# VITA-Group/mm-hand

Measured on AMD Instinct MI355X. Metric: 256x256 hand images/sec (G+D step), higher is better.
Workload: dtype f32; 1 GPU; RHD-shaped 256x256, per-GPU batch 32, fp32 (Winograd F(6x6,3x3) on the 3x3 stack), G(9 PATBlocks, ngf64)+D_PB+D_PP+L1/perceptual/GAN+Adam, --norm instance, dropout on; VGG19[:4] weights: random-init (seed 1234): NOT the reference's pretrained objective; global_batch=32, parallelism=dp1

## Files before the change

### include/mmhand_hip.h

```cpp
#ifndef MMHAND_HIP_H
#define MMHAND_HIP_H

#include <stddef.h>
#include <stdint.h>

#ifdef __cplusplus
extern "C" {
#endif
#pragma GCC visibility push(default)

typedef void* mmh_stream_t;

enum { MMH_PAD_ZERO = 0, MMH_PAD_REFLECT = 1 };
enum { MMH_ACT_NONE = 0, MMH_ACT_RELU = 1, MMH_ACT_TANH = 2 };
enum { MMH_F32 = 0, MMH_BF16 = 1, MMH_FP16 = 2 };

typedef struct mmh_conv_desc {
    int32_t B, H, W;
    int32_t Cin, Cout;
    int32_t kh, kw;
    int32_t stride;
    int32_t pad;
    int32_t pad_mode;
    int32_t Ho, Wo;
// ... 1 lines not shown
    int32_t dtype;
} mmh_conv_desc;

const char* mmh_last_error(void);
int mmh_version(void);
int mmh_set_option(const char* key, int value);


int mmh_conv2d_fprop(const mmh_conv_desc* d, const void* x, const void* w,
                     const void* bias, void* y, int act, mmh_stream_t s);

int mmh_conv2d_fprop_stats_chunks(const mmh_conv_desc* d);
int mmh_conv2d_fprop_stats(const mmh_conv_desc* d, const void* x, const void* w, const void* bias,
                           void* y, void* stats, mmh_stream_t s);
int mmh_dgrad_s2_halo_supported(const mmh_conv_desc* d, int dx_cs);

int mmh_conv2d_dgrad(const mmh_conv_desc* d, const void* dy, const void* w,
                     void* dx, int dx_cs, mmh_stream_t s);

size_t mmh_conv2d_dgrad_folded_ws_bytes(const mmh_conv_desc* d);
int mmh_conv2d_dgrad_folded(const mmh_conv_desc* d, const void* dy, const void* w,
                            void* dx, void* ws, size_t ws_bytes, mmh_stream_t s);

int mmh_wino_weights(const void* w, int Cin, int Cout, int flip_transpose, int tile, int dtype,
                     void* U, mmh_stream_t s);
int mmh_wino_input(const void* x, int B, int H, int W, int C, int reflect, int tile, int dtype,
                   void* V, mmh_stream_t s);
int mmh_wino_dy(const void* dy, int B, int H, int W, int C, int tile, int dtype, void* Yh,
                mmh_stream_t s);
int mmh_wino_input_dy(const void* dy, int B, int H, int W, int C, int tile, int dtype, void* V,
// ... 390 lines not shown
```

### mmhand_amd/csrc/common.h

```cpp
#pragma once
#include <hip/hip_runtime.h>
#include <cstdarg>
#include <cstdio>
#include <cstdint>
#include "../../include/mmhand_hip.h"

namespace mmh {

char* err_buf();
int fail(const char* fmt, ...);

inline int check_launch(const char* what) {
    hipError_t e = hipGetLastError();
    if (e != hipSuccess) return fail("%s: %s", what, hipGetErrorString(e));
    return 0;
}

inline hipStream_t as_stream(mmh_stream_t s) { return reinterpret_cast<hipStream_t>(s); }

inline int64_t cdiv(int64_t a, int64_t b) { return (a + b - 1) / b; }

int wino6_weights(const float* w, float* U, int Cin, int Cout, int flip_transpose, hipStream_t st);
int wino6_weights_multi(const long long* table, int n, long long total_blocks, hipStream_t st);
int wino6_input(const float* x, float* V, int B, int H, int W, int C, int reflect, int xcd, hipStream_t st);
// ... 5 lines not shown
                        const uint32_t* drows, hipStream_t st);
int wino6_input_dy_normbwd(const float* g, const float* x, float* V, float* Yh, int B, int H, int W, int C, int xcd,
                           int fold, const float* mean, const float* invstd, const float* gamma, const float* s1,
                           const float* s2, double count, const float* scale, const float* shift,
                           const uint32_t* drows, int groups, int relu, float drop_p, hipStream_t st);
int wino6_input_dy(const float* dy, float* V, float* Yh, int B, int H, int W, int C, int xcd, int fold,
                   hipStream_t st);
int wino6_dw(const float* dU, float* dw, int Cin, int Cout, int accumulate, hipStream_t st);
bool wgrad_lp16t_supported(const mmh_conv_desc* d);
int wgrad_lp16t_splits(const mmh_conv_desc* d);
int launch_wgrad_lp16t(const mmh_conv_desc* d, const void* x16, const void* dy16, float* slab, const void* zeros,
                       hipStream_t st);
bool dgrad_s2_halo_ok(const mmh_conv_desc* d, int dx_cs, int act);
int launch_dgrad_s2_halo(const mmh_conv_desc* d, const void* dy, const void* w, const void* bias, void* dx, int dx_cs,
                         int act, hipStream_t st);
extern int g_dgrad_s2_halo, g_dgrad_s2_dbg;
bool wgrad_s2_strip_ok(const mmh_conv_desc* d);
size_t wgrad_s2_strip_ws_bytes(const mmh_conv_desc* d);
int launch_wgrad_s2_strip(const mmh_conv_desc* d, const void* x, const void* dy, void* dw, void* ws, size_t ws_bytes,
                          int accumulate, hipStream_t st);
extern int g_wgrad_s2_strip;
bool stem_f32_ok(const mmh_conv_desc* d);
int stem_f32_stats_chunks(const mmh_conv_desc* d);
int launch_stem_f32(const mmh_conv_desc* d, const void* x, const void* w, const void* bias, void* y, int act, float* stats,
                    hipStream_t st);
extern int g_stem_f32, g_stem_f32_dbg, g_stem_f32_levels;
bool wino_wgrad_dma_ok(int64_t tiles, int Cin, int Cout, int nbatch);
size_t wino_wgrad_dma_ws_bytes(int64_t tiles, int Cin, int Cout, int nbatch);
int launch_wino_wgrad_dma(const float* V, const float* Yh, int64_t tiles, int Cin, int Cout, int nbatch, float* ws, float* dU,
                          hipStream_t st);
extern int g_wino_wgrad_dma;
// ... 28 lines not shown
```

### mmhand_amd/csrc/conv_igemm.hip

```cpp
#include <algorithm>
#include <cstring>
#include "device_prims.h"

namespace {
using namespace mmh::dev;

typedef __bf16 bf16x4 __attribute__((ext_vector_type(4)));
typedef __bf16 bf16x2 __attribute__((ext_vector_type(2)));
typedef _Float16 f16x4 __attribute__((ext_vector_type(4)));
typedef _Float16 f16x2 __attribute__((ext_vector_type(2)));
__device__ __forceinline__ bf16x4 to_bf16x4(float4 v) {
    bf16x4 r;
    r[0] = (__bf16)v.x; r[1] = (__bf16)v.y; r[2] = (__bf16)v.z; r[3] = (__bf16)v.w;
    return r;
}
template <bool H16>
__device__ __forceinline__ bf16x4 to_lp4(float4 v) {
    if (H16) {
        f16x4 r;
        r[0] = (_Float16)v.x; r[1] = (_Float16)v.y; r[2] = (_Float16)v.z; r[3] = (_Float16)v.w;
        return __builtin_bit_cast(bf16x4, r);
    }
    return to_bf16x4(v);
}
// ... 2915 lines not shown
    if (!strcmp(key, "wino6_vec")) { mmh::g_wino6_vec = value; return 0; }
    if (!strcmp(key, "lp16_shape")) { mmh::g_lp16_shape = value; return 0; }
    if (!strcmp(key, "lp16_s2f")) { mmh::g_lp16_s2f = value; return 0; }
    if (!strcmp(key, "lp16_persist")) { mmh::g_lp16_persist = value; return 0; }
    if (!strcmp(key, "lp16_tap_inner")) { mmh::g_lp16_tap_inner = value; return 0; }
    if (!strcmp(key, "pw_v2")) { mmh::g_pw_v2 = value; return 0; }
    if (!strcmp(key, "col_chunks") && value > 0) { mmh::g_col_chunks = value; return 0; }
    if (!strcmp(key, "row_chunks") && value > 0) { mmh::g_row_chunks = value; return 0; }
    if (!strcmp(key, "dgrad_s2_halo")) { mmh::g_dgrad_s2_halo = value; return 0; }
    if (!strcmp(key, "wgrad_s2_strip")) { mmh::g_wgrad_s2_strip = value; return 0; }
    if (!strcmp(key, "stem_f32")) { mmh::g_stem_f32 = value; return 0; }
    if (!strcmp(key, "wino_wgrad_dma")) { mmh::g_wino_wgrad_dma = value; return 0; }
    if (!strcmp(key, "stem_f32_dbg")) { mmh::g_stem_f32_dbg = value; return 0; }
    if (!strcmp(key, "slab_reduce_par")) { mmh::g_slab_reduce_par = value; return 0; }
    if (!strcmp(key, "dgrad_s2_dbg")) { mmh::g_dgrad_s2_dbg = value; return 0; }
    if (!strcmp(key, "lp16_dbg")) { mmh::g_lp16_dbg = value; return 0; }
    if (!strcmp(key, "lp16_wgrad_ring")) { mmh::g_lp16_wgrad_ring = value; return 0; }
    if (!strcmp(key, "lp16_wgrad_s2")) { mmh::g_lp16_wgrad_s2 = value; return 0; }
    if (!strcmp(key, "border_bn64")) { g_border_bn64 = value; return 0; }
    if (!strcmp(key, "wino_gemm_occ")) { g_wino_gemm_occ = value; return 0; }
    if (!strcmp(key, "wino_gemm_levels")) { g_wino_gemm_levels = value; return 0; }
    if (!strcmp(key, "wino_gemm_bn")) { g_wino_gemm_bn = value; return 0; }
    if (!strcmp(key, "wino_bf16_occ")) { g_wino_bf16_occ = value; return 0; }
    if (!strcmp(key, "wino_bf16_bk")) { g_wino_bf16_bk = value; return 0; }
    if (!strcmp(key, "wino_wgrad_bn256")) { g_wino_wgrad_bn256 = value; return 0; }
    if (!strcmp(key, "wino_wgrad_slots")) { g_wino_wgrad_slots = value; return 0; }
    return mmh::fail("mmh_set_option: unknown key '%s'", key);
}

int mmh_conv2d_fprop(const mmh_conv_desc* d, const void* x, const void* w, const void* bias,
// ... 466 lines not shown
```

### mmhand_amd/csrc/dgrad_s2.hip

```cpp
#include <algorithm>
#include <type_traits>
#include "device_prims.h"

namespace mmh { int g_dgrad_s2_halo = 1; int g_dgrad_s2_dbg = 0; }

namespace {
using namespace mmh::dev;

constexpr int KC = 64;
constexpr int TH = 8, TW = 16;
constexpr int HWD = TW + 1;
constexpr int HPIX_REAL = (TH + 1) * HWD;
constexpr int PIXB = KC * 4;
constexpr int NT = 512;
constexpr int PPR = NT * 16 / PIXB;
constexpr int HROUNDS = (HPIX_REAL + PPR - 1) / PPR;
constexpr int HALO_B = HROUNDS * PPR * PIXB;
constexpr int lds_bytes(int ntn) { return 2 * HALO_B + 2 * (64 * ntn) * PIXB; }

__device__ char g_zero_line[128];
constexpr int wait_vm(int n) { return (n & 15) | ((n >> 4) << 14) | 0x0070; }
template <int V> using IC = std::integral_constant<int, V>;
constexpr int tap_of(int i) { return i == 0 ? 4 : i == 1 ? 3 : i == 2 ? 5 : i == 3 ? 1 : i == 4 ? 7 : i == 5 ? 0 : i == 6 ? 2 : i == 7 ? 6 : 8; }

struct DgradS2KP {
    const float* dy;
    const float* w;
    const float* bias;
    float* dx;
    int B, Ho, Wo, dx_cs, act;
    int TX, TY, tiles, per_xcd, slots, dbg;
};


template <int CTRL>
__device__ __forceinline__ float quad_xchg(float v) {
    return __builtin_bit_cast(float, __builtin_amdgcn_update_dpp(0, __builtin_bit_cast(int, v), CTRL, 0xf, 0xf, true));
}
__device__ __forceinline__ f32x4 quad_transpose(float v0, float v1, float v2, float v3, bool odd, bool hi) {
    const float r01 = quad_xchg<0xB1>(odd ? v0 : v1), r23 = quad_xchg<0xB1>(odd ? v2 : v3);
    const float p0x = odd ? r01 : v0, p0y = odd ? v1 : r01;
    const float p1x = odd ? r23 : v2, p1y = odd ? v3 : r23;
    const float sx = quad_xchg<0x4E>(hi ? p0x : p1x), sy = quad_xchg<0x4E>(hi ? p0y : p1y);
    f32x4 o;
    o[0] = hi ? sx : p0x;
    o[1] = hi ? sy : p0y;
    o[2] = hi ? p1x : sx;
    o[3] = hi ? p1y : sy;
    return o;
}

template <bool EPI, int NTN, int KQ>
__global__ void __launch_bounds__(NT, 1) dgrad_s2_kernel(const DgradS2KP p) {
    constexpr int CI = 64 * NTN, CO = KC * KQ;
    constexpr int WST_B = CI * PIXB;
    constexpr int WROUNDS = CI / PPR;
    constexpr int NQ = 9 * KQ;
    constexpr int NSC = 4 * NTN;
    static_assert(KQ % 2 == 0, "the halo buffers alternate per chunk and a tile must start on buffer 0");
    extern __shared__ __attribute__((aligned(1024))) char smem[];
    const int tid = threadIdx.x;
    const int lane = tid & 63, wave = __builtin_amdgcn_readfirstlane(tid >> 6);
    const int r = lane & 31, kg = lane >> 5;
    const int pg = wave & 3, ch = wave >> 2;
    const unsigned lds0 = lds_addr_of(smem);
    const unsigned wdst = __builtin_amdgcn_readfirstlane(lds0 + (unsigned)wave * 1024u);
    const int xcd = blockIdx.x & 7, slot = blockIdx.x >> 3;
    const int t_end = min(p.tiles, (xcd + 1) * p.per_xcd);
// ... 62 lines not shown
    bool counted = false;
    for (; tile < t_end; tile += p.slots) {
        const int b = tile / tpi;
        const int trem = tile - b * tpi;
        const int ty = trem / p.TX, tx = trem - ty * p.TX;
        const bool full = ty * TH + TH <= p.Ho && tx * TW + TW <= p.Wo;
        wq = p.w;
        asm volatile("" : "+s"(wq));
        f32x16 acc[4][NTN];
#pragma unroll
        for (int c = 0; c < 4; ++c)
#pragma unroll
            for (int nt = 0; nt < NTN; ++nt)
#pragma unroll
                for (int i = 0; i < 16; ++i) acc[c][nt][i] = 0.f;

        float* const tile_o = p.dx + ((size_t)(b * H + 2 * (ty * TH + 2 * pg)) * W + 2 * tx * TW) * (size_t)p.dx_cs;
        const int pw_room = p.Wo - tx * TW, ph_room = p.Ho - (ty * TH + 2 * pg);
        auto store_class = [&](auto cc) {
            constexpr int c = decltype(cc)::value;
            if (p.dbg & 1) return;
#pragma unroll
            for (int g = 0; g < 4; ++g) {
                float* const o = tile_o + (size_t)(2 * (g >> 1) + (c >> 1)) * rs + (size_t)((16 * (g & 1) + (c & 1)) * p.dx_cs);
                const bool ok = full || ((g >> 1) < ph_room && 8 * (g & 1) + pw_lane < pw_room);
#pragma unroll
                for (int nt = 0; nt < NTN; ++nt) {
                    f32x4 v = quad_transpose(acc[c][nt][4 * g], acc[c][nt][4 * g + 1], acc[c][nt][4 * g + 2], acc[c][nt][4 * g + 3],
                                             odd, hi);
                    if (EPI) {
#pragma unroll
                        for (int e = 0; e < 4; ++e) v[e] = fmaxf(v[e] + bv[nt][e], relu_floor);
                    }
                    if (p.dbg & 16) asm volatile("" ::"v"(v[0]), "v"(v[1]), "v"(v[2]), "v"(v[3]), "v"(st_lane));
                    else if (ok) *reinterpret_cast<f32x4*>(o + st_lane + 32 * nt) = v;
                }
            }
        };

        auto phase = [&](auto qc) {
            constexpr int q = decltype(qc)::value;
            constexpr int kq = q / 9, ti = q - 9 * kq, tap = tap_of(ti);
            constexpr int kh = tap / 3, kw = tap - 3 * (tap / 3);
            constexpr int dh = kh == 0 ? 1 : 0, dw = kw == 0 ? 1 : 0;
            constexpr int cls = (kh != 1 ? 2 : 0) + (kw != 1 ? 1 : 0);
            constexpr bool last = kq == KQ - 1;
            constexpr bool after_halo = q > 0 && (q - 1) % 9 == 0;
            constexpr bool after_store = (q == 0) || (kq == KQ - 1 && (ti == 2 || ti == 4 || ti == 6));
            asm volatile("" ::: "memory");
            if (after_halo) {
                __builtin_amdgcn_s_waitcnt(wait_vm(HROUNDS));
            } else if (after_store) {
                if (q == 0 ? counted : full) __builtin_amdgcn_s_waitcnt(wait_vm(NSC));
                else __builtin_amdgcn_s_waitcnt(wait_vm(0));
            } else {
                __builtin_amdgcn_s_waitcnt(wait_vm(0));
            }
            __builtin_amdgcn_s_barrier();
            asm volatile("" ::: "memory");
            if (!(p.dbg & 4)) issue_w(q + 1 < NQ ? q + 1 : 0);
            if (ti == 0 && !(p.dbg & 2)) {
                if (last) issue_halo(tile + p.slots, 0);
                else issue_halo(tile, kq + 1);
            }
            if (last && ch == 0) {
                if (ti == 1) store_class(IC<0>{});
                if (ti == 3) store_class(IC<1>{});
                if (ti == 5) store_class(IC<2>{});
            }
            unsigned ab = a_lane[dh][dw] + (unsigned)((kq & 1) * HALO_B);
            unsigned bb = b_lane + (unsigned)((q & 1) * WST_B);
            asm volatile("" : "+v"(ab), "+v"(bb));
            f32x4 af = lds_f4(ab), bf[NTN];
#pragma unroll
            for (int nt = 0; nt < NTN; ++nt) bf[nt] = lds_f4(bb + (unsigned)(nt * 32 * PIXB));
#pragma unroll
            for (int kc = 0; kc < 8; ++kc) {
                f32x4 an, bn[NTN];
                if (kc + 1 < 8) {
                    an = lds_f4(ab ^ (unsigned)((kc + 1) << 5));
// ... 17 lines not shown
                if (ti == 5) store_class(IC<2>{});
            }
        };
        auto chunk = [&](auto kc_) {
            constexpr int q0 = 9 * decltype(kc_)::value;
            phase(IC<q0>{}); phase(IC<q0 + 1>{}); phase(IC<q0 + 2>{}); phase(IC<q0 + 3>{}); phase(IC<q0 + 4>{});
            phase(IC<q0 + 5>{}); phase(IC<q0 + 6>{}); phase(IC<q0 + 7>{}); phase(IC<q0 + 8>{});
        };
        chunk(IC<0>{});
        chunk(IC<1>{});
        if constexpr (KQ == 4) {
            chunk(IC<2>{});
            chunk(IC<3>{});
        }
        store_class(IC<3>{});
        counted = full && !(p.dbg & 1);
    }
}

}

namespace mmh {

bool dgrad_s2_halo_ok(const mmh_conv_desc* d, int dx_cs, int act) {
    return g_dgrad_s2_halo && act != MMH_ACT_TANH && d->dtype == MMH_F32 && d->kh == 3 && d->kw == 3 && d->stride == 2 && d->pad == 1 &&
           d->pad_mode == MMH_PAD_ZERO && ((d->Cin == 64 && d->Cout == 128) || (d->Cin == 128 && d->Cout == 256)) &&
           d->y_cs == d->Cout && d->H == 2 * d->Ho && d->W == 2 * d->Wo && dx_cs >= d->Cin && dx_cs % 4 == 0 &&
           (size_t)d->B * d->H * d->W * dx_cs < (1ull << 31);
}

template <bool EPI, int NTN, int KQ>
static int launch_t(const DgradS2KP& p, hipStream_t st) {
    static int ready = -1;
    if (ready != 0) {
        hipError_t e = hipFuncSetAttribute(reinterpret_cast<const void*>(dgrad_s2_kernel<EPI, NTN, KQ>),
                                           hipFuncAttributeMaxDynamicSharedMemorySize, lds_bytes(NTN));
        if (e != hipSuccess) return fail("dgrad_s2: %s", hipGetErrorString(e));
        ready = 0;
    }
    hipLaunchKernelGGL((dgrad_s2_kernel<EPI, NTN, KQ>), dim3(8 * p.slots), dim3(NT), lds_bytes(NTN), st, p);
    return check_launch("dgrad_s2_kernel");
}

int launch_dgrad_s2_halo(const mmh_conv_desc* d, const void* dy, const void* w, const void* bias, void* dx, int dx_cs,
                         int act, hipStream_t st) {
    DgradS2KP p{};
    p.dy = static_cast<const float*>(dy);
    p.w = static_cast<const float*>(w);
    p.bias = static_cast<const float*>(bias);
    p.dx = static_cast<float*>(dx);
    p.B = d->B; p.Ho = d->Ho; p.Wo = d->Wo; p.dx_cs = dx_cs; p.act = act;
    p.TY = (d->Ho + TH - 1) / TH;
    p.TX = (d->Wo + TW - 1) / TW;
    p.tiles = p.B * p.TX * p.TY;
    p.per_xcd = (p.tiles + 7) / 8;
    static int cus = 0;
    if (!cus) {
        int dev = 0;
        hipDeviceProp_t prop;
        if (hipGetDevice(&dev) != hipSuccess || hipGetDeviceProperties(&prop, dev) != hipSuccess)
            return fail("dgrad_s2: cannot query the device");
        cus = prop.multiProcessorCount;
    }
    p.slots = std::max(1, std::min(cus / 8, p.per_xcd));
    p.dbg = g_dgrad_s2_dbg;
    const bool epi = bias || act != MMH_ACT_NONE;
    if (d->Cin == 64) return epi ? launch_t<true, 1, 2>(p, st) : launch_t<false, 1, 2>(p, st);
    return epi ? launch_t<true, 2, 4>(p, st) : launch_t<false, 2, 4>(p, st);
}

}

extern "C" int mmh_dgrad_s2_halo_supported(const mmh_conv_desc* d, int dx_cs) {
    return d && mmh::dgrad_s2_halo_ok(d, dx_cs, MMH_ACT_NONE) ? 1 : 0;
}
```

### mmhand_amd/lib.py

```python
import ctypes as C
import os

_HERE = os.path.dirname(os.path.abspath(__file__))
LIB_PATH = os.environ.get("MMH_LIB_PATH") or os.path.join(_HERE, "libmmhand_hip.so")

PAD_ZERO, PAD_REFLECT = 0, 1
ACT_NONE, ACT_RELU, ACT_TANH = 0, 1, 2
F32, BF16, FP16 = 0, 1, 2
U8 = 3


class ConvDesc(C.Structure):
    _fields_ = [(n, C.c_int32) for n in (
        "B", "H", "W", "Cin", "Cout", "kh", "kw", "stride", "pad", "pad_mode",
        "Ho", "Wo", "x_cs", "y_cs", "dtype")]


class PlaneSrc(C.Structure):
    _fields_ = [("ptr", C.c_void_p), ("C", C.c_int32),
                ("sb", C.c_int64), ("sc", C.c_int64), ("sh", C.c_int64), ("sw", C.c_int64)]


class ImageSrc(C.Structure):
    _fields_ = [("ptr", C.c_void_p), ("dtype", C.c_int32), ("scale", C.c_float), ("offset", C.c_float),
# ... 57 lines not shown
    "mmh_prep_weights_fp16": (_i, [_vp, _i, _i, _i, _vp, _vp, _vp]),
    "mmh_prep_weights_fp16_flat": (_i, [_vp, _i, _i, _i, _vp, _vp]),
    "mmh_cvt_lp16": (_i, [_vp, _i64, _i, _vp, _vp]),
    "mmh_conv_lp16_supported": (_i, [_DP, _i]),
    "mmh_conv_lp16": (_i, [_DP, _i, _vp, _vp, _vp, _vp, _i, _i, _vp, _vp]),
    "mmh_conv_lp16_stats_chunks": (_i, [_DP]),
    "mmh_conv_lp16_fprop_stats": (_i, [_DP, _vp, _vp, _vp, _vp, _vp, _vp, _vp]),
    "mmh_conv_stem16_stats_chunks": (_i, [_DP, _i]),
    "mmh_conv_stem16_stats": (_i, [_DP, _vp, _i, _vp, _vp, _vp, _vp, _vp, _vp]),
    "mmh_lp16_pad_cvt": (_i, [_vp, _i64, _i, _i, _i, _vp, _vp]),
    "mmh_prep_weights_lp16_flat8": (_i, [_vp, _i, _i, _i, _i, _i, _vp, _vp]),
    "mmh_conv_lp16_flat_supported": (_i, [_DP, _i]),
    "mmh_conv_lp16_flat": (_i, [_DP, _vp, _i, _vp, _vp, _vp, _i, _i, _vp, _vp]),
    "mmh_conv_stem16_supported": (_i, [_DP, _i]),
    "mmh_dgrad_s2_halo_supported": (_i, [_DP, _i]),
    "mmh_conv_stem16_weights_bytes": (_sz, [_i]),
    "mmh_prep_weights_stem16": (_i, [_vp, _i, _i, _i, _vp, _vp]),
    "mmh_conv_stem16_weights_bytes_k": (_sz, [_i, _i]),
    "mmh_prep_weights_stem16_k": (_i, [_vp, _i, _i, _i, _i, _vp, _vp]),
    "mmh_conv_stem16": (_i, [_DP, _vp, _i, _vp, _vp, _vp, _i, _i, _vp, _vp]),
    "mmh_wgrad_stem_lp16_supported": (_i, [_DP, _i]),
    "mmh_wgrad_stem_lp16_ws_bytes": (_sz, [_DP, _i]),
    "mmh_wgrad_stem_lp16": (_i, [_DP, _vp, _i, _vp, _vp, _vp, _sz, _i, _vp, _vp]),
    "mmh_conv7_head_wgrad_lp16_supported": (_i, [_DP]),
    "mmh_conv7_head_wgrad_lp16_ws_bytes": (_sz, [_DP]),
    "mmh_conv7_head_wgrad_lp16": (_i, [_DP, _vp, _vp, _vp, _vp, _sz, _i, _vp, _vp]),
    "mmh_wgrad_lp16_flat_supported": (_i, [_DP, _i]),
    "mmh_wgrad_lp16_flat_ws_bytes": (_sz, [_DP, _i]),
    "mmh_wgrad_lp16_flat": (_i, [_DP, _vp, _i, _i, _vp, _vp, _vp, _sz, _i, _vp, _vp]),
    "mmh_conv7_head_dgrad_lp16_supported": (_i, [_DP]),
# ... 120 lines not shown
```

### mmhand_amd/ops.py

```python
import ctypes as C
import os
import weakref

import torch

from . import lib as L


def _ptr(t):
    return None if t is None else C.c_void_p(t.data_ptr())


_raw_stream = getattr(torch._C, "_cuda_getCurrentRawStream", None)
_raw_device = getattr(torch._C, "_cuda_getDevice", None)


def _stream():
    if _raw_stream is not None and _raw_device is not None:
        return C.c_void_p(_raw_stream(_raw_device()))
    return C.c_void_p(torch.cuda.current_stream().cuda_stream)


def _chk(t, name="tensor"):
    if not (t.is_cuda and t.dtype == torch.float32 and t.is_contiguous()):
# ... 704 lines not shown
            return raw_conv3x3_lp16(dy16, w, None, True, L.ACT_NONE, bf16, 2, out16=out16, addend=addend, nbr=nbr)
        dx = raw_conv3x3_lp16(dy16, w, None, False, L.ACT_NONE, bf16, 1, out16=out16, addend=addend,
                              nbr=None if reflect else nbr)
        if reflect:
            ws = torch.empty(L.load().mmh_conv2d_dgrad_border_ws_bytes(C.byref(d)) // 4 + 4, dtype=torch.float32,
                             device=dx.device)
            L.call("mmh_conv2d_dgrad_border", C.byref(d), _ptr(dy16), _ptr(bf16_weights(w, bf16)[0]), _ptr(dx), _ptr(ws),
                   ws.numel() * 4, 3, 1 | (2 if out16 else 0), _stream())
        return dx
    if bf16 and not reflect and lp16g_ok(d, 1, bf16):
        return raw_conv_lp16g(d, 1, dy16 if dy16 is not None else lp16_twin(dy, bf16), w, None, L.ACT_NONE, bf16,
                              out16=out16)
    if bf16 and Cout % 64 == 0:
        d.dtype = _dt(bf16)
        w = bf16_weights(w, bf16)[0]
    dx = _empty((B, H, W_, Cin), dy)
    nbytes = L.load().mmh_conv2d_dgrad_folded_ws_bytes(C.byref(d))
    ws = _ws(nbytes, dy) if nbytes else None
    L.call("mmh_conv2d_dgrad_folded", C.byref(d), _ptr(dy), _ptr(w), _ptr(dx), _ptr(ws),
           ws.numel() * 4 if ws is not None else 0, _stream())
    _count_desc("mfma", d)
    return dx


def raw_conv_wgrad(x, dy, k, stride, pad, reflect, bf16=False, out=None):
    B, H, W_, Cin = x.shape
    Cout = dy.shape[3]
    if not x.is_contiguous() and not (bf16 and x.dtype != torch.float32 and lp16_wgrad_ok(Cin, Cout, k, stride, pad)):
        x = x.contiguous()
    if x.is_contiguous():
# ... 109 lines not shown
        return g


USE_LP16_FOLD = os.environ.get("MMH_LP16_FOLD", "1") != "0"


def lp16_v2_ok(Cin, Cout, k, stride, pad, mode):
    n = Cout if mode == 0 else Cin
    return USE_LP16_V2 and k == 3 and stride == 1 and pad == 1 and Cin % 64 == 0 and Cout % 64 == 0 and n % 256 == 0


USE_NBR = os.environ.get("MMH_FUSE_NORM_BWD_REDUCE", "1") != "0"
NBR_MIN_C = int(os.environ.get("MMH_NBR_MIN_C", "256"))


class NormBwdSite:
    __slots__ = ("x", "bits", "mean", "invstd", "groups", "drop_p", "g", "s1", "s2")

    def __init__(self, x, bits, mean, invstd, groups, drop_p):
        self.x, self.bits, self.mean, self.invstd, self.groups, self.drop_p = x, bits, mean, invstd, groups, drop_p
        self.g = self.s1 = self.s2 = None


_nbr_sites = {}


def nbr_site_put(a16, site):
    while len(_nbr_sites) >= 8:
        _nbr_sites.pop(next(iter(_nbr_sites)))
    _nbr_sites[a16.data_ptr()] = (a16, site)
# ... 543 lines not shown
        ctx.g_defer = bool(g_defer)
        ctx.skip_db = bool(null_bias_grad and EXACT_NULL_BIAS_GRAD)
        ctx.bias_p = bias
        B, H, W_, Cin = x.shape
        ctx.dx_channels = dx_channels
        wt = _wino_tile(B, H, W_, Cin, w.shape[3], w.shape[0], stride, pad, bf16)
        ctx.cfg = (stride, pad, reflect, act, bias is not None, bf16)
        ctx.x_shape = tuple(x.shape)
        ctx.wino_V = 0
        ctx.lp16 = False
        ctx.x_lp = x16 is not None
        ctx.y_lp = bool(y_lp)
        k = w.shape[0]
        ctx.stem16 = ctx.head16 = False
        ctx.nbr = nbr_site_take(x16) if (x16 is not None and torch.is_tensor(x16)) else None
        if pro is not None:
            assert wt == 6 and not bf16 and x16 is None and not y_lp, "a deferred norm needs the fp32 F(6x6,3x3) path"
            if KEEP_WINOGRAD_INPUT and ctx.needs_input_grad[1]:
                y, V = raw_conv_fprop_wino(x, w, bias, reflect, act, wt, keep_V=True, pro=pro)
                ctx.wino_V = wt
                ctx.save_for_backward(V, w, y if act != L.ACT_NONE else None)
                return y
            assert not ctx.needs_input_grad[1], "a deferred norm in front of a trainable conv needs MMH_WINOGRAD_KEEP_INPUT=1"
            y = raw_conv_fprop_wino(x, w, bias, reflect, act, wt, pro=pro)
            ctx.save_for_backward(None, w, y if act != L.ACT_NONE else None)
            return y
        chain = bool(bf16) and lp16_chain_ok(Cin, w.shape[3], k, stride, pad, reflect, bf16)
        head16 = bool(bf16) and k == 7 and not y_lp and not dx_channels and pro is None \
            and head16_ok(B, H, W_, Cin, w.shape[3], k, stride, pad, reflect, bf16)
        if x16 is not None:
# ... 160 lines not shown
                db = _finish_param_grad(raw_colsum(g.numel() // g.shape[3], g.shape[3], g, out=bt_), bt_)
            return _tok_add(dx, addend), dw, db, None, None, None, None, None, None, None, None, None, None, None, None, None
        if (not WINOGRAD_FPROP and FUSE_WINO6_BWD and not bf16 and not ctx.wino_V and not ctx.dx_channels
                and ctx.needs_input_grad[0] and ctx.needs_input_grad[1] and x is not None and x.dtype == torch.float32
                and _wino_tile(*ctx.x_shape, w.shape[3], w.shape[0], stride, pad, bf16, "dgrad") == 6
                and _wino_tile(*ctx.x_shape, w.shape[3], w.shape[0], stride, pad, bf16, "wgrad") == 6):
            Bx, Hx, Wx, Cx = ctx.x_shape
            V = _empty((64, Bx * (-(-Hx // 6)) * (-(-Wx // 6)), Cx), x)
            L.call("mmh_wino_input", _ptr(x), Bx, Hx, Wx, Cx, int(bool(reflect)), 6, L.F32, _ptr(V), _stream())
            dx, dw = raw_conv_bwd_wino6(g, w, ctx.x_shape, reflect, V, dw_out=wt_)
            dw = _finish_param_grad(dw, wt_)
            if want_db:
                db = _finish_param_grad(raw_colsum(g.numel() // g.shape[3], g.shape[3], g, out=bt_), bt_)
            return _tok_add(dx, addend), dw, db, None, None, None, None, None, None, None, None, None, None, None, None, None
        if ctx.needs_input_grad[0]:
            dx = raw_conv_dgrad(g, w, ctx.x_shape, stride, pad, reflect, bf16, ctx.dx_channels)
        if ctx.needs_input_grad[1]:
            if ctx.wino_V:
                dw = _finish_param_grad(raw_conv_wgrad_wino(None, g, reflect, ctx.wino_V, V=x, bf16=bf16, out=wt_), wt_)
            else:
                dw = _finish_param_grad(raw_conv_wgrad(x, g, w.shape[0], stride, pad, reflect, bf16, out=wt_), wt_)
        if want_db:
            db = _finish_param_grad(raw_colsum(g.numel() // g.shape[3], g.shape[3], g, out=bt_), bt_)
        return _tok_add(dx, addend), dw, db, None, None, None, None, None, None, None, None, None, None, None, None, None


class ConvT2dFn(torch.autograd.Function):

    @staticmethod
    def forward(ctx, x, w, bias, bf16=False, x16=None, y_lp=False, null_bias_grad=False):
        ctx.set_materialize_grads(False)
        _dp_use(ctx.needs_input_grad, w, bias)
        ctx.skip_db = bool(null_bias_grad and EXACT_NULL_BIAS_GRAD)
        ctx.bias_p = bias
        ctx.has_bias = bias is not None
        ctx.bf16 = bf16
        ctx.x_lp = x16 is not None
        ctx.y_lp = bool(y_lp)
        ctx.x_shape = tuple(x.shape)
        chain = bool(bf16) and convT_lp16_ok(x.shape[3], w.shape[2], bf16)
        if x16 is not None or y_lp:
            assert chain, "16-bit edges of a ConvTranspose2d need 16-bit kernels for all three passes"
        if chain:
            if x16 is None:
                x16 = lp16_twin(x, bf16)
            y = raw_convT_fprop(x16, w, bias, L.ACT_NONE, bf16, out16=bool(y_lp))
            ctx.lp16 = True
            ctx.save_for_backward(x16, w)
            if y_lp:
                ctx.mark_non_differentiable(y)
                return lp_proxy(y.shape, y.device), y
            return y
        ctx.lp16 = False
        y = raw_convT_fprop(x, w, bias, L.ACT_NONE, bf16)
# ... 328 lines not shown
        return lp_proxy(x.shape, x.device), scale, shift, drows
    masked = bool(relu or drop_p > 0)
    twin_lp = want_twin if (want_twin and not out_lp and norm_twin_ok(x.shape[3])) else 0
    r = raw_scale_shift_act(x, scale, shift, residual, relu, drop_p, seed, mask, keep_bits=masked, out_lp=out_lp,
                            twin_lp=twin_lp)
    r = r if isinstance(r, tuple) else (r,)
    out, kb, twin = r[0], (r[1] if masked else None), (r[-1] if twin_lp else None)
    ctx.cfg = (groups, rows, count, bool(relu), float(drop_p), sync_group,
               residual is not None)
    ctx.save_for_backward(x, kb, mean, invstd, gamma)
    ctx.nbr_site = None
    if (USE_NBR and out_lp and masked and residual is None and x.dtype != torch.float32 and x.shape[3] >= NBR_MIN_C
            and x.shape[3] % 256 == 0):
        ctx.nbr_site = NormBwdSite(x, kb, mean, invstd, groups, float(drop_p))
        nbr_site_put(out, ctx.nbr_site)
    if want_twin and not out_lp:
        if twin is not None:
            ctx.mark_non_differentiable(twin)
        return out, twin
    if out_lp:
        if residual is not None:
            raise RuntimeError("NormActFn: a 16-bit output together with a residual is not supported")
        ctx.mark_non_differentiable(out)
        return lp_proxy(x.shape, x.device), out
    return (out,)


USE_NORM_BWD_PLANE = os.environ.get("MMH_NORM_BWD_PLANE", "0") == "1"


# ... 4 lines not shown
        x, dbits, mean, invstd, gamma, scale, shift, drows = ctx.saved_tensors
        g = g.contiguous()
        Cc = x.shape[3]
        ws = _ws(L.load().mmh_norm_bwd_ws_bytes(groups, rows, Cc), x)
        s1, s2 = sums_out if sums_out is not None else (_empty((groups, Cc), x), _empty((groups, Cc), x))
        L.call("mmh_norm_bwd_reduce_rc", _ptr(g), _ptr(x), _ptr(mean), _ptr(invstd), _ptr(scale), _ptr(shift),
               _ptr(dbits), groups, rows, Cc, int(relu), drop_p, _ptr(s1), _ptr(s2), _ptr(ws), ws.numel() * 4, _stream())
        return g, s1, s2
    x, out, mean, invstd, gamma = ctx.saved_tensors
    if has_res and relu:
        raise RuntimeError("NormActFn: residual together with ReLU is not on the reference path")
    g = lp_grad_in(g, "NormActFn") if ctx.out_lp else g.contiguous()
    Cc = x.shape[3]
    masked = 2 if (relu or drop_p > 0) else 0
    site = getattr(ctx, "nbr_site", None)
    if site is not None and site.g is g and site.s1 is not None:
        s1, s2 = site.s1, site.s2
        site.g = site.s1 = site.s2 = None
        if sums_out is not None:
            sums_out[0].copy_(s1.view_as(sums_out[0]))
            sums_out[1].copy_(s2.view_as(sums_out[1]))
            s1, s2 = sums_out
        return g, s1, s2
    s1, s2 = sums_out if sums_out is not None else (_empty((groups, Cc), x), _empty((groups, Cc), x))
    if (USE_NORM_BWD_PLANE and sync_group is None and x.dtype != torch.float32 and g.dtype in (torch.float32, x.dtype)
            and L.load().mmh_norm_bwd_fused_supported(groups, rows, Cc, masked, _tdt(g), _tdt(x))):
        dx = torch.empty_like(x)
        L.call("mmh_norm_bwd_fused", _ptr(g), _ptr(out), _ptr(x), _ptr(mean), _ptr(invstd), _ptr(gamma), float(count),
               groups, rows, Cc, masked, drop_p, _ptr(s1), _ptr(s2), _ptr(dx), _tdt(g), _tdt(x), _tdt(dx), _stream())
        ctx.fused_dx = dx
        return g, s1, s2
    ws = _ws(L.load().mmh_norm_bwd_ws_bytes(groups, rows, Cc), x)
    L.call("mmh_norm_bwd_reduce", _ptr(g), _ptr(out), _ptr(x), _ptr(mean), _ptr(invstd), groups,
# ... 710 lines not shown
```

Before: 120.7 images/s.

## Fuse instance-norm backward reductions into the fp32 stride-2 dgrad halo kernel

```diff
diff --git a/include/mmhand_hip.h b/include/mmhand_hip.h
--- a/include/mmhand_hip.h
+++ b/include/mmhand_hip.h
@@ -39,6 +39,10 @@
 int mmh_conv2d_fprop_stats(const mmh_conv_desc* d, const void* x, const void* w, const void* bias,
                            void* y, void* stats, mmh_stream_t s);
 int mmh_dgrad_s2_halo_supported(const mmh_conv_desc* d, int dx_cs);
+size_t mmh_conv2d_dgrad_s2_nbr_ws_bytes(const mmh_conv_desc* d, int groups);
+int mmh_conv2d_dgrad_s2_nbr(const mmh_conv_desc* d, const void* dy, const void* w, void* dx, const void* x,
+                            const void* keep_bits, const void* mean, const void* invstd, int groups, int masked,
+                            float drop_p, void* s1, void* s2, void* ws, size_t ws_bytes, mmh_stream_t s);
 
 int mmh_conv2d_dgrad(const mmh_conv_desc* d, const void* dy, const void* w,
                      void* dx, int dx_cs, mmh_stream_t s);
diff --git a/mmhand_amd/csrc/common.h b/mmhand_amd/csrc/common.h
--- a/mmhand_amd/csrc/common.h
+++ b/mmhand_amd/csrc/common.h
@@ -43,7 +43,7 @@
 bool dgrad_s2_halo_ok(const mmh_conv_desc* d, int dx_cs, int act);
 int launch_dgrad_s2_halo(const mmh_conv_desc* d, const void* dy, const void* w, const void* bias, void* dx, int dx_cs,
                          int act, hipStream_t st);
-extern int g_dgrad_s2_halo, g_dgrad_s2_dbg;
+extern int g_dgrad_s2_halo, g_dgrad_s2_dbg, g_dgrad_s2_nbr;
 bool wgrad_s2_strip_ok(const mmh_conv_desc* d);
 size_t wgrad_s2_strip_ws_bytes(const mmh_conv_desc* d);
 int launch_wgrad_s2_strip(const mmh_conv_desc* d, const void* x, const void* dy, void* dw, void* ws, size_t ws_bytes,
diff --git a/mmhand_amd/csrc/conv_igemm.hip b/mmhand_amd/csrc/conv_igemm.hip
--- a/mmhand_amd/csrc/conv_igemm.hip
+++ b/mmhand_amd/csrc/conv_igemm.hip
@@ -2953,6 +2953,7 @@
     if (!strcmp(key, "stem_f32_dbg")) { mmh::g_stem_f32_dbg = value; return 0; }
     if (!strcmp(key, "slab_reduce_par")) { mmh::g_slab_reduce_par = value; return 0; }
     if (!strcmp(key, "dgrad_s2_dbg")) { mmh::g_dgrad_s2_dbg = value; return 0; }
+    if (!strcmp(key, "dgrad_s2_nbr")) { mmh::g_dgrad_s2_nbr = value; return 0; }
     if (!strcmp(key, "lp16_dbg")) { mmh::g_lp16_dbg = value; return 0; }
     if (!strcmp(key, "lp16_wgrad_ring")) { mmh::g_lp16_wgrad_ring = value; return 0; }
     if (!strcmp(key, "lp16_wgrad_s2")) { mmh::g_lp16_wgrad_s2 = value; return 0; }
diff --git a/mmhand_amd/csrc/dgrad_s2.hip b/mmhand_amd/csrc/dgrad_s2.hip
--- a/mmhand_amd/csrc/dgrad_s2.hip
+++ b/mmhand_amd/csrc/dgrad_s2.hip
@@ -2,7 +2,7 @@
 #include <type_traits>
 #include "device_prims.h"
 
-namespace mmh { int g_dgrad_s2_halo = 1; int g_dgrad_s2_dbg = 0; }
+namespace mmh { int g_dgrad_s2_halo = 1; int g_dgrad_s2_dbg = 0; int g_dgrad_s2_nbr = 1; }
 
 namespace {
 using namespace mmh::dev;
@@ -30,6 +30,13 @@
     float* dx;
     int B, Ho, Wo, dx_cs, act;
     int TX, TY, tiles, per_xcd, slots, dbg;
+    const float* nx;
+    const uint8_t* nbits;
+    const float* nmean;
+    const float* ninv;
+    float* npart;
+    int ngrp_b;
+    float ndsc;
 };
 
 
@@ -50,8 +57,9 @@
     return o;
 }
 
-template <bool EPI, int NTN, int KQ>
+template <bool EPI, int NTN, int KQ, bool NBR = false>
 __global__ void __launch_bounds__(NT, 1) dgrad_s2_kernel(const DgradS2KP p) {
+    static_assert(!(EPI && NBR), "the norm-backward sums belong to a plain dgrad");
     constexpr int CI = 64 * NTN, CO = KC * KQ;
     constexpr int WST_B = CI * PIXB;
     constexpr int WROUNDS = CI / PPR;
@@ -144,9 +152,31 @@
             for (int nt = 0; nt < NTN; ++nt)
 #pragma unroll
                 for (int i = 0; i < 16; ++i) acc[c][nt][i] = 0.f;
+        f32x4 xr[4][NTN], mu[NTN], is[NTN], s1[NTN], s2[NTN];
+        unsigned kb[4][NTN];
+#pragma unroll
+        for (int nt = 0; nt < NTN; ++nt) s1[nt] = s2[nt] = (f32x4){0.f, 0.f, 0.f, 0.f};
 
         float* const tile_o = p.dx + ((size_t)(b * H + 2 * (ty * TH + 2 * pg)) * W + 2 * tx * TW) * (size_t)p.dx_cs;
         const int pw_room = p.Wo - tx * TW, ph_room = p.Ho - (ty * TH + 2 * pg);
+        const unsigned tile_e = (unsigned)(tile_o - p.dx);
+        auto load_x = [&](auto cc) {
+            constexpr int c = decltype(cc)::value;
+#pragma unroll
+            for (int g = 0; g < 4; ++g) {
+                const unsigned eo = tile_e + (unsigned)(2 * (g >> 1) + (c >> 1)) * (unsigned)rs + (unsigned)((16 * (g & 1) + (c & 1)) * CI) + st_lane;
+                const bool ok = full || ((g >> 1) < ph_room && 8 * (g & 1) + pw_lane < pw_room);
+#pragma unroll
+                for (int nt = 0; nt < NTN; ++nt) {
+                    xr[g][nt] = (f32x4){0.f, 0.f, 0.f, 0.f};
+                    kb[g][nt] = 0u;
+                    if (ok) {
+                        xr[g][nt] = *reinterpret_cast<const f32x4*>(p.nx + eo + 32 * nt);
+                        kb[g][nt] = p.nbits ? (unsigned)p.nbits[(eo >> 2) + 8 * nt] : 0xfu;
+                    }
+                }
+            }
+        };
         auto store_class = [&](auto cc) {
             constexpr int c = decltype(cc)::value;
             if (p.dbg & 1) return;
@@ -161,6 +191,14 @@
                     if (EPI) {
 #pragma unroll
                         for (int e = 0; e < 4; ++e) v[e] = fmaxf(v[e] + bv[nt][e], relu_floor);
+                    }
+                    if (NBR) {
+#pragma unroll
+                        for (int e = 0; e < 4; ++e) {
+                            const float dz = (kb[g][nt] >> e) & 1u ? v[e] * p.ndsc : 0.f;
+                            s2[nt][e] += dz * ((xr[g][nt][e] - mu[nt][e]) * is[nt][e]);
+                            s1[nt][e] += dz;
+                        }
                     }
                     if (p.dbg & 16) asm volatile("" ::"v"(v[0]), "v"(v[1]), "v"(v[2]), "v"(v[3]), "v"(st_lane));
                     else if (ok) *reinterpret_cast<f32x4*>(o + st_lane + 32 * nt) = v;
@@ -181,19 +219,38 @@
             if (after_halo) {
                 __builtin_amdgcn_s_waitcnt(wait_vm(HROUNDS));
             } else if (after_store) {
-                if (q == 0 ? counted : full) __builtin_amdgcn_s_waitcnt(wait_vm(NSC));
+                if (q == 0 ? counted : (full && !(NBR && ch == 0))) __builtin_amdgcn_s_waitcnt(wait_vm(NSC + (NBR && q == 0 ? 2 * NTN : 0)));
                 else __builtin_amdgcn_s_waitcnt(wait_vm(0));
             } else {
                 __builtin_amdgcn_s_waitcnt(wait_vm(0));
             }
             __builtin_amdgcn_s_barrier();
             asm volatile("" ::: "memory");
+            if constexpr (NBR) {
+                if (kq == KQ - 2 && ti == 8) {
+                    const int grp = p.ngrp_b ? b : 0;
+#pragma unroll
+                    for (int nt = 0; nt < NTN; ++nt) {
+                        mu[nt] = *reinterpret_cast<const f32x4*>(p.nmean + grp * CI + n4 + 32 * nt);
+                        is[nt] = *reinterpret_cast<const f32x4*>(p.ninv + grp * CI + n4 + 32 * nt);
+                    }
+                    load_x(IC<0>{});
+                }
+                if (last && ti == 2) load_x(IC<1>{});
+                if (last && ti == 4) load_x(IC<2>{});
+                if (last && ti == 7) load_x(IC<3>{});
+                if (last && ch == 0) {
+                    if (ti == 1) store_class(IC<0>{});
+                    if (ti == 3) store_class(IC<1>{});
+                    if (ti == 5) store_class(IC<2>{});
+                }
+            }
             if (!(p.dbg & 4)) issue_w(q + 1 < NQ ? q + 1 : 0);
             if (ti == 0 && !(p.dbg & 2)) {
                 if (last) issue_halo(tile + p.slots, 0);
                 else issue_halo(tile, kq + 1);
             }
-            if (last && ch == 0) {
+            if (!NBR && last && ch == 0) {
                 if (ti == 1) store_class(IC<0>{});
                 if (ti == 3) store_class(IC<1>{});
                 if (ti == 5) store_class(IC<2>{});
@@ -241,6 +298,27 @@
             chunk(IC<3>{});
         }
         store_class(IC<3>{});
+        if constexpr (NBR) {
+#pragma unroll
+            for (int nt = 0; nt < NTN; ++nt)
+#pragma unroll
+                for (int e = 0; e < 4; ++e) {
+                    float a = s1[nt][e], c2 = s2[nt][e];
+                    a += quad_xchg<0xB1>(a); c2 += quad_xchg<0xB1>(c2);
+                    a += quad_xchg<0x4E>(a); c2 += quad_xchg<0x4E>(c2);
+                    a += __builtin_bit_cast(float, __builtin_amdgcn_ds_bpermute((lane ^ 32) << 2, __builtin_bit_cast(int, a)));
+                    c2 += __builtin_bit_cast(float, __builtin_amdgcn_ds_bpermute((lane ^ 32) << 2, __builtin_bit_cast(int, c2)));
+                    s1[nt][e] = a; s2[nt][e] = c2;
+                }
+            if ((lane & 35) == 0) {
+                float* const o = p.npart + ((size_t)(tile * 4 + pg) * 2) * CI + n4;
+#pragma unroll
+                for (int nt = 0; nt < NTN; ++nt) {
+                    *reinterpret_cast<f32x4*>(o + 32 * nt) = s1[nt];
+                    *reinterpret_cast<f32x4*>(o + CI + 32 * nt) = s2[nt];
+                }
+            }
+        }
         counted = full && !(p.dbg & 1);
     }
 }
@@ -256,22 +334,21 @@
            (size_t)d->B * d->H * d->W * dx_cs < (1ull << 31);
 }
 
-template <bool EPI, int NTN, int KQ>
+template <bool EPI, int NTN, int KQ, bool NBR = false>
 static int launch_t(const DgradS2KP& p, hipStream_t st) {
     static int ready = -1;
     if (ready != 0) {
-        hipError_t e = hipFuncSetAttribute(reinterpret_cast<const void*>(dgrad_s2_kernel<EPI, NTN, KQ>),
+        hipError_t e = hipFuncSetAttribute(reinterpret_cast<const void*>(dgrad_s2_kernel<EPI, NTN, KQ, NBR>),
                                            hipFuncAttributeMaxDynamicSharedMemorySize, lds_bytes(NTN));
         if (e != hipSuccess) return fail("dgrad_s2: %s", hipGetErrorString(e));
         ready = 0;
     }
-    hipLaunchKernelGGL((dgrad_s2_kernel<EPI, NTN, KQ>), dim3(8 * p.slots), dim3(NT), lds_bytes(NTN), st, p);
+    hipLaunchKernelGGL((dgrad_s2_kernel<EPI, NTN, KQ, NBR>), dim3(8 * p.slots), dim3(NT), lds_bytes(NTN), st, p);
     return check_launch("dgrad_s2_kernel");
 }
 
-int launch_dgrad_s2_halo(const mmh_conv_desc* d, const void* dy, const void* w, const void* bias, void* dx, int dx_cs,
-                         int act, hipStream_t st) {
-    DgradS2KP p{};
+static int fill_params(DgradS2KP& p, const mmh_conv_desc* d, const void* dy, const void* w, const void* bias, void* dx, int dx_cs,
+                       int act) {
     p.dy = static_cast<const float*>(dy);
     p.w = static_cast<const float*>(w);
     p.bias = static_cast<const float*>(bias);
@@ -291,6 +368,13 @@
     }
     p.slots = std::max(1, std::min(cus / 8, p.per_xcd));
     p.dbg = g_dgrad_s2_dbg;
+    return 0;
+}
+
+int launch_dgrad_s2_halo(const mmh_conv_desc* d, const void* dy, const void* w, const void* bias, void* dx, int dx_cs,
+                         int act, hipStream_t st) {
+    DgradS2KP p{};
+    if (int rc = fill_params(p, d, dy, w, bias, dx, dx_cs, act)) return rc;
     const bool epi = bias || act != MMH_ACT_NONE;
     if (d->Cin == 64) return epi ? launch_t<true, 1, 2>(p, st) : launch_t<false, 1, 2>(p, st);
     return epi ? launch_t<true, 2, 4>(p, st) : launch_t<false, 2, 4>(p, st);
@@ -298,6 +382,42 @@
 
 }
 
+extern "C" size_t mmh_conv2d_dgrad_s2_nbr_ws_bytes(const mmh_conv_desc* d, int groups) {
+    if (!d || d->B <= 0 || d->Ho <= 0 || d->Wo <= 0 || !mmh::g_dgrad_s2_nbr || !mmh::dgrad_s2_halo_ok(d, d->Cin, MMH_ACT_NONE) || d->Cin != 64 || d->x_cs != d->Cin ||
+        (groups != 1 && groups != d->B))
+        return 0;
+    const size_t tiles = (size_t)d->B * ((d->Ho + TH - 1) / TH) * ((d->Wo + TW - 1) / TW);
+    return tiles * 4 * 2 * d->Cin * sizeof(float);
+}
+
+extern "C" int mmh_conv2d_dgrad_s2_nbr(const mmh_conv_desc* d, const void* dy, const void* w, void* dx, const void* x,
+                                       const void* keep_bits, const void* mean, const void* invstd, int groups, int masked,
+                                       float drop_p, void* s1, void* s2, void* ws, size_t ws_bytes, mmh_stream_t s) {
+    MMH_REQUIRE(d != nullptr, "mmh_conv2d_dgrad_s2_nbr: NULL descriptor");
+    const size_t need = mmh_conv2d_dgrad_s2_nbr_ws_bytes(d, groups);
+    MMH_REQUIRE(need > 0, "mmh_conv2d_dgrad_s2_nbr: needs the halo kernel (mmh_dgrad_s2_halo_supported), a dense dx, groups 1 | B "
+                          "and mmh_set_option(\"dgrad_s2_nbr\") != 0 (ask mmh_conv2d_dgrad_s2_nbr_ws_bytes)");
+    MMH_REQUIRE(dy && w && dx && x && mean && invstd && s1 && s2 && ws, "mmh_conv2d_dgrad_s2_nbr: NULL buffer");
+    MMH_REQUIRE((masked == 0 || masked == 2) && (!masked || keep_bits) && drop_p >= 0.f && drop_p < 1.f && (masked || drop_p == 0.f),
+                "mmh_conv2d_dgrad_s2_nbr: masked must be 0 or 2 (keep bits, 4 per float4), 0 <= drop_p < 1, dropout needs the bits");
+    MMH_REQUIRE(ws_bytes >= need && ((uintptr_t)ws & 15) == 0 && ((uintptr_t)x & 15) == 0 && ((uintptr_t)mean & 15) == 0 &&
+                    ((uintptr_t)invstd & 15) == 0,
+                "mmh_conv2d_dgrad_s2_nbr: workspace too small (%zu < %zu) or a buffer not 16-byte aligned", ws_bytes, need);
+    MMH_REQUIRE(!mmh::g_dgrad_s2_dbg, "mmh_conv2d_dgrad_s2_nbr: not under the timing ablations (dgrad_s2_dbg)");
+    hipStream_t st = mmh::as_stream(s);
+    DgradS2KP p{};
+    if (int rc = mmh::fill_params(p, d, dy, w, nullptr, dx, d->Cin, MMH_ACT_NONE)) return rc;
+    p.nx = static_cast<const float*>(x);
+    p.nbits = masked ? static_cast<const uint8_t*>(keep_bits) : nullptr;
+    p.nmean = static_cast<const float*>(mean);
+    p.ninv = static_cast<const float*>(invstd);
+    p.npart = static_cast<float*>(ws);
+    p.ngrp_b = groups == d->B && groups != 1;
+    p.ndsc = 1.f / (1.f - drop_p);
+    if (int rc = mmh::launch_t<false, 1, 2, true>(p, st)) return rc;
+    return mmh_norm_bwd_sums_final(ws, groups, d->Cin, p.tiles * 4 / groups, s1, s2, s);
+}
+
 extern "C" int mmh_dgrad_s2_halo_supported(const mmh_conv_desc* d, int dx_cs) {
     return d && mmh::dgrad_s2_halo_ok(d, dx_cs, MMH_ACT_NONE) ? 1 : 0;
 }
diff --git a/mmhand_amd/lib.py b/mmhand_amd/lib.py
--- a/mmhand_amd/lib.py
+++ b/mmhand_amd/lib.py
@@ -95,6 +95,8 @@
     "mmh_conv_lp16_flat": (_i, [_DP, _vp, _i, _vp, _vp, _vp, _i, _i, _vp, _vp]),
     "mmh_conv_stem16_supported": (_i, [_DP, _i]),
     "mmh_dgrad_s2_halo_supported": (_i, [_DP, _i]),
+    "mmh_conv2d_dgrad_s2_nbr_ws_bytes": (_sz, [_DP, _i]),
+    "mmh_conv2d_dgrad_s2_nbr": (_i, [_DP, _vp, _vp, _vp, _vp, _vp, _vp, _vp, _i, _i, _f, _vp, _vp, _vp, _sz, _vp]),
     "mmh_conv_stem16_weights_bytes": (_sz, [_i]),
     "mmh_prep_weights_stem16": (_i, [_vp, _i, _i, _i, _vp, _vp]),
     "mmh_conv_stem16_weights_bytes_k": (_sz, [_i, _i]),
diff --git a/mmhand_amd/ops.py b/mmhand_amd/ops.py
--- a/mmhand_amd/ops.py
+++ b/mmhand_amd/ops.py
@@ -742,6 +742,20 @@
     if bf16 and Cout % 64 == 0:
         d.dtype = _dt(bf16)
         w = bf16_weights(w, bf16)[0]
+    if (nbr is not None and not bf16 and not reflect and k == 3 and stride == 2 and pad == 1 and Cout == 2 * Cin
+            and dy.dtype == torch.float32 and tuple(nbr.x.shape) == (B, H, W_, Cin) and nbr.x.dtype == torch.float32
+            and nbr.x.is_contiguous() and not any(t.data_ptr() % 16 for t in (nbr.x, nbr.mean, nbr.invstd))):
+        nbytes = nbr_s2_ws_bytes(x_shape, nbr.groups)
+        if nbytes:
+            dx = _empty((B, H, W_, Cin), dy)
+            ws = _ws(nbytes, dy)
+            s1, s2 = _empty((nbr.groups, Cin), dy), _empty((nbr.groups, Cin), dy)
+            L.call("mmh_conv2d_dgrad_s2_nbr", C.byref(d), _ptr(dy), _ptr(w), _ptr(dx), _ptr(nbr.x), _ptr(nbr.bits), _ptr(nbr.mean),
+                   _ptr(nbr.invstd), nbr.groups, 2 if nbr.bits is not None else 0, float(nbr.drop_p), _ptr(s1), _ptr(s2), _ptr(ws),
+                   ws.numel() * 4, _stream())
+            nbr.g, nbr.s1, nbr.s2 = dx, s1, s2
+            _count_desc("mfma", d)
+            return dx
     dx = _empty((B, H, W_, Cin), dy)
     nbytes = L.load().mmh_conv2d_dgrad_folded_ws_bytes(C.byref(d))
     ws = _ws(nbytes, dy) if nbytes else None
@@ -881,6 +895,17 @@
 NBR_MIN_C = int(os.environ.get("MMH_NBR_MIN_C", "256"))
 
 
+USE_NBR_S2 = os.environ.get("MMH_FUSE_NORM_BWD_REDUCE_S2", "1") != "0"
+
+
+def nbr_s2_ws_bytes(x_shape, groups):
+    B, H, W_, Cc = x_shape
+    if not USE_NBR_S2 or H % 2 or W_ % 2:
+        return 0
+    d = conv_desc(B, H, W_, Cc, 2 * Cc, 3, 2, 1, False)
+    return int(L.load().mmh_conv2d_dgrad_s2_nbr_ws_bytes(C.byref(d), groups))
+
+
 class NormBwdSite:
     __slots__ = ("x", "bits", "mean", "invstd", "groups", "drop_p", "g", "s1", "s2")
 
@@ -1454,6 +1479,11 @@
         k = w.shape[0]
         ctx.stem16 = ctx.head16 = False
         ctx.nbr = nbr_site_take(x16) if (x16 is not None and torch.is_tensor(x16)) else None
+        if x16 is None and _nbr_sites and x.dtype == torch.float32:
+            site = nbr_site_take(x)
+            if (site is not None and not bf16 and k == 3 and stride == 2 and pad == 1 and not reflect and pro is None
+                    and not dx_channels and res_tok is None and act == L.ACT_NONE):
+                ctx.nbr = site
         if pro is not None:
             assert wt == 6 and not bf16 and x16 is None and not y_lp, "a deferred norm needs the fp32 F(6x6,3x3) path"
             if KEEP_WINOGRAD_INPUT and ctx.needs_input_grad[1]:
@@ -1644,7 +1674,8 @@
                 db = _finish_param_grad(raw_colsum(g.numel() // g.shape[3], g.shape[3], g, out=bt_), bt_)
             return _tok_add(dx, addend), dw, db, None, None, None, None, None, None, None, None, None, None, None, None, None
         if ctx.needs_input_grad[0]:
-            dx = raw_conv_dgrad(g, w, ctx.x_shape, stride, pad, reflect, bf16, ctx.dx_channels)
+            dx = raw_conv_dgrad(g, w, ctx.x_shape, stride, pad, reflect, bf16, ctx.dx_channels,
+                                nbr=ctx.nbr if (addend is None and not ctx.dx_channels) else None)
         if ctx.needs_input_grad[1]:
             if ctx.wino_V:
                 dw = _finish_param_grad(raw_conv_wgrad_wino(None, g, reflect, ctx.wino_V, V=x, bf16=bf16, out=wt_), wt_)
@@ -1668,6 +1699,8 @@
         ctx.x_lp = x16 is not None
         ctx.y_lp = bool(y_lp)
         ctx.x_shape = tuple(x.shape)
+        if x16 is None and _nbr_sites:
+            nbr_site_take(x)
         chain = bool(bf16) and convT_lp16_ok(x.shape[3], w.shape[2], bf16)
         if x16 is not None or y_lp:
             assert chain, "16-bit edges of a ConvTranspose2d need 16-bit kernels for all three passes"
@@ -2026,6 +2059,10 @@
             and x.shape[3] % 256 == 0):
         ctx.nbr_site = NormBwdSite(x, kb, mean, invstd, groups, float(drop_p))
         nbr_site_put(out, ctx.nbr_site)
+    elif (USE_NBR_S2 and not out_lp and x16 is None and twin is None and residual is None and sync_group is None
+          and x.dtype == torch.float32 and x.is_cuda and nbr_s2_ws_bytes(x.shape, groups)):
+        ctx.nbr_site = NormBwdSite(x, kb, mean, invstd, groups, float(drop_p))
+        nbr_site_put(out, ctx.nbr_site)
     if want_twin and not out_lp:
         if twin is not None:
             ctx.mark_non_differentiable(twin)
@@ -2060,9 +2097,11 @@
     Cc = x.shape[3]
     masked = 2 if (relu or drop_p > 0) else 0
     site = getattr(ctx, "nbr_site", None)
-    if site is not None and site.g is g and site.s1 is not None:
+    taken = site is not None and site.g is g and site.s1 is not None
+    if site is not None:
         s1, s2 = site.s1, site.s2
         site.g = site.s1 = site.s2 = None
+    if taken:
         if sums_out is not None:
             sums_out[0].copy_(s1.view_as(sums_out[0]))
             sums_out[1].copy_(s2.view_as(sums_out[1]))
```

Result: no change. 121.1 images/s (median of 6 runs) (+0.4%).
